# georghess/neurad-studio

Measured on NVIDIA H100. Metric: rays/sec (camera+lidar), higher is better.
Workload: dtype f32

## Files before the change

### neurad-studio_b200/csrc/b200nerf.cu

```cuda
#include <cuda_runtime.h>

#include <cstdio>
#include <cstring>
#include <new>
#include <string>
#include <vector>

#include "../../include/b200nerf.h"
#include "nff_device.h"
#include "nff_lane.h"
#include "rgb_decoder.cuh"
#include "modules.cuh"

using namespace nff;

static thread_local std::string g_err;
static int fail(int code, const std::string& msg) {
  g_err = msg;
  return code;
}
#define CUDA_TRY(expr)                                                                                   \
  do {                                                                                                   \
    cudaError_t e_ = (expr);                                                                             \
    if (e_ != cudaSuccess)                                                                               \
// ... 108 lines not shown
  mlp.stage = reinterpret_cast<float*>(smem_tc + kTcBytes) + group * kTcStageFloats;
  mlp.bar_id = 1 + group;
  const int64_t stride = (int64_t)gridDim.x * WARPS;
  for (int64_t base = (int64_t)blockIdx.x * WARPS; base < P.n_rays; base += stride) {
    const int64_t ray = base + warp;
    const bool active = ray < P.n_rays;
    render_ray(P, *ws, mlp, active ? ray : P.n_rays - 1, active);
  }
}



__device__ __forceinline__ int64_t lane_units(const RenderParams& P) {
  const int W = P.rays.image_width;
  if (W <= 0) return (P.n_rays + kLaneThreads - 1) / kLaneThreads;
  constexpr int kTileH = kLaneThreads / 32;
  const int64_t H = (P.n_rays + W - 1) / W;
  return (int64_t)((W + 31) / 32) * ((H + kTileH - 1) / kTileH);
}
__device__ __forceinline__ bool lane_unit_ray(const RenderParams& P, int64_t unit, int tid, int64_t* ray_out) {
  const int W = P.rays.image_width;
  int64_t ray, fallback;
  bool active;
  if (W > 0) {
    constexpr int kTileH = kLaneThreads / 32;
    const int64_t H = (P.n_rays + W - 1) / W, tiles_x = (W + 31) / 32;
    const int warp = tid >> 5, lane_ = tid & 31;
    const int64_t px = (unit % tiles_x) * 32 + (warp & 3) * 8 + (lane_ & 7);
    const int64_t py = (unit / tiles_x) * kTileH + (warp >> 2) * 4 + (lane_ >> 3);
    ray = py * W + px;
    active = px < W && ray < P.n_rays;
    fallback = (py < H ? py : H - 1) * W + (px < W ? px : W - 1);
  } else {
    ray = unit * kLaneThreads + tid;
    active = ray < P.n_rays;
    fallback = P.n_rays - 1;
  }
  if (fallback >= P.n_rays) fallback = P.n_rays - 1;
  *ray_out = active ? ray : fallback;
  return active;
}

__device__ __forceinline__ int64_t lane_patches(const RenderParams& P) {
  return P.rays.image_width > 0 ? lane_units(P) * (kLaneThreads / 32) : (P.n_rays + 31) / 32;
}
__device__ __forceinline__ bool lane_patch_ray(const RenderParams& P, int64_t patch, int lane_, int64_t* ray_out) {
  constexpr int kPatchesPerUnit = kLaneThreads / 32;
  return lane_unit_ray(P, patch / kPatchesPerUnit, (int)(patch % kPatchesPerUnit) * 32 + lane_, ray_out);
}

#ifndef NFF_SAMPLE_CTAS
#define NFF_SAMPLE_CTAS 2
#endif
template <int LAYOUT>
__global__ void __launch_bounds__(kLaneThreads, NFF_SAMPLE_CTAS) nff_sample_lane_kernel(const __grid_constant__ RenderParams P,
                                                                                        float* __restrict__ scratch,
                                                                                        float* __restrict__ handoff) {
  const int tid = threadIdx.x, warp = __shfl_sync(0xffffffffu, (int)(threadIdx.x >> 5), 0), lane_ = tid & 31;
  const LaneScratch sc = lane_scratch_of(scratch, blockIdx.x);
  constexpr int kPPU = kLaneThreads / 32;
  const int64_t n_patches = lane_patches(P);
  const int64_t full_rounds = n_patches / kPPU / gridDim.x;
  const int64_t r0 = full_rounds * gridDim.x * kPPU, rest = n_patches - r0;
  const int64_t p0 = r0 + rest * blockIdx.x / gridDim.x, p1 = r0 + rest * (blockIdx.x + 1) / gridDim.x;
  for (int64_t it = 0;; ++it) {
    int64_t patch;
    if (it < full_rounds) {
      patch = (it * gridDim.x + blockIdx.x) * kPPU + warp;
    } else {
      patch = p0 + warp + (it - full_rounds) * kPPU;
      if (patch >= p1) break;
    }
    int64_t ray;
    const bool active = lane_patch_ray(P, patch, lane_, &ray);
    const LaneRay R = lane_ray_setup(P, sc, tid, ray);
    float* col = active ? handoff + ray : sc.bins2 + tid;
    sample_ray_lane<LAYOUT>(P, sc, R, tid, ray, active, col, active ? P.n_rays : (int64_t)kLaneThreads);
  }
}

template <int LAYOUT>
__global__ void __launch_bounds__(kLaneThreads, kLaneCtasPerSm) nff_shade_lane_kernel(const __grid_constant__ RenderParams P,
                                                                                      float* __restrict__ scratch,
                                                                                      const float* __restrict__ handoff) {
  extern __shared__ __align__(128) unsigned char smem_shade[];
  TcShared* tcs = reinterpret_cast<TcShared*>(smem_shade);
  const int tid = threadIdx.x, warp = __shfl_sync(0xffffffffu, (int)(threadIdx.x >> 5), 0), group = warp >> 2;
  tc_stage_weights(*tcs, P.main_mlp_nn, tid, kLaneThreads, true);
  tc::fence_async_smem();
  __syncthreads();
  MlpLaneTc mlp;
  mlp.t = tcs;
  mlp.panel_ = reinterpret_cast<float*>(smem_shade + kTcBytes);
  mlp.bar_id = 1 + group;
  const LaneScratch sc = lane_scratch_of(scratch, blockIdx.x);
  mlp.sh_tcnn = LAYOUT;
  constexpr int kPPU = kLaneThreads / 32;
  const int64_t n_patches = lane_patches(P);
  const int64_t full_rounds = n_patches / kPPU / gridDim.x;
  const int64_t r0 = full_rounds * gridDim.x * kPPU;
  const int64_t rest_groups = (n_patches - r0 + 3) / 4;
  const int64_t g0 = rest_groups * blockIdx.x / gridDim.x, g1 = rest_groups * (blockIdx.x + 1) / gridDim.x;
  for (int64_t it = 0;; ++it) {
    int64_t patch;
    if (it < full_rounds) {
      patch = (it * gridDim.x + blockIdx.x) * kPPU + warp;
    } else {
      const int64_t gu = g0 + group + (it - full_rounds) * (kLaneThreads / 128);
      if (gu >= g1) break;
      patch = r0 + gu * 4 + (warp & 3);
    }
    int64_t ray;
    const bool active = lane_patch_ray(P, patch, tid & 31, &ray);
    const LaneRay R = lane_ray_setup(P, sc, tid, ray);
    shade_ray_lane<MlpLaneTc, LAYOUT>(P, sc, R, mlp, tid, ray, active, handoff + ray, P.n_rays);
  }
}

__global__ void __launch_bounds__(kLaneThreads, kLaneCtasPerSm) nff_render_lane_kernel(const __grid_constant__ RenderParams P,
                                                                          float* __restrict__ scratch) {
  extern __shared__ __align__(128) unsigned char smem_lane[];
  TcShared* tcs = reinterpret_cast<TcShared*>(smem_lane);
  const int tid = threadIdx.x, warp = __shfl_sync(0xffffffffu, (int)(threadIdx.x >> 5), 0), group = warp >> 2;
  tc_stage_weights(*tcs, P.main_mlp_nn, tid, kLaneThreads, true);
  tc::fence_async_smem();
  __syncthreads();
  MlpLaneTc mlp;
  mlp.t = tcs;
  mlp.panel_ = reinterpret_cast<float*>(smem_lane + kTcBytes);
  mlp.bar_id = 1 + group;
  const LaneScratch sc = lane_scratch_of(scratch, blockIdx.x);
// ... 634 lines not shown
static void offset_rays(RenderParams& Q, int64_t start, int fdim) {
  if (start == 0) return;
  adv(Q.rays.origins, 3 * start); adv(Q.rays.directions, 3 * start); adv(Q.rays.pixel_area, start);
  adv(Q.rays.times, start); adv(Q.rays.nears, start); adv(Q.rays.fars, start);
  adv(Q.rays.sensor_idx, start); adv(Q.rays.is_lidar, start);
  adv(Q.out.features, (int64_t)fdim * start); adv(Q.out.depth, start); adv(Q.out.accumulation, start);
  adv(Q.out.prop_depth_0, start); adv(Q.out.prop_depth_1, start);
  b200nerf_trace& t = Q.trace;
  adv(t.prop_weights_0, kS0 * start); adv(t.prop_weights_1, kS1 * start);
  adv(t.bins_s_1, (kS1 + 1) * start); adv(t.bins_e_1, (kS1 + 1) * start);
  adv(t.bins_s_2, (kS2 + 1) * start); adv(t.bins_e_2, (kS2 + 1) * start);
  adv(t.inds_1, (kS1 + 1) * start); adv(t.inds_2, (kS2 + 1) * start);
  adv(t.sdf, kS2 * start); adv(t.alpha, kS2 * start); adv(t.field_feature, (int64_t)kS2 * kNff * start);
  adv(t.weights, kS2 * start);
  adv(t.actor_id_0, kS0 * start); adv(t.actor_id_1, kS1 * start); adv(t.actor_id_main, kS2 * start);
  Q.peers.row_offset += start;
}


extern "C" {

const char* b200nerf_last_error(void) { return g_err.c_str(); }
int b200nerf_version(void) { return B200NERF_VERSION; }

int b200nerf_create(int device_ordinal, b200nerf_ctx** out) {
  REQUIRE(out != nullptr, "out is NULL");
  int n = 0;
  CUDA_TRY(cudaGetDeviceCount(&n));
  REQUIRE(device_ordinal >= 0 && device_ordinal < n, "device ordinal out of range");
  DeviceGuard g(device_ordinal);
  cudaDeviceProp prop;
  CUDA_TRY(cudaGetDeviceProperties(&prop, device_ordinal));
  if (prop.major != 9 || prop.minor != 0)
    return fail(B200NERF_ERR_UNSUPPORTED, "libb200nerf is built for sm_90a only (found sm_" +
                                              std::to_string(prop.major) + std::to_string(prop.minor) + ")");
  b200nerf_ctx* c = new (std::nothrow) b200nerf_ctx();
  REQUIRE(c != nullptr, "out of host memory");
  c->device = device_ordinal;
  c->sm_count = prop.multiProcessorCount;
  CUDA_TRY(cudaFuncSetAttribute(nff_render_kernel<kRenderWarps>, cudaFuncAttributeMaxDynamicSharedMemorySize,
                                (int)((kMainMlpFloats * 4 + 15) / 16 * 16 + kRenderWarps * sizeof(WarpShared))));
  CUDA_TRY(cudaFuncSetAttribute(nff_render_tc_kernel<kRenderWarps>, cudaFuncAttributeMaxDynamicSharedMemorySize,
                                (int)(tc_smem_bytes(kRenderWarps * 32) + kRenderWarps * sizeof(WarpSharedTc))));
  CUDA_TRY(cudaMalloc((void**)&c->d_status, sizeof(int)));
  CUDA_TRY(cudaMemset(c->d_status, 0, sizeof(int)));
  CUDA_TRY(cudaFuncSetAttribute(nff_render_lane_kernel, cudaFuncAttributeMaxDynamicSharedMemorySize,
                                (int)lane_tc_smem_bytes()));
  c->lane_ctas = c->sm_count * (kLaneCtasPerSm > NFF_SAMPLE_CTAS ? kLaneCtasPerSm : NFF_SAMPLE_CTAS);
  CUDA_TRY(cudaMalloc((void**)&c->d_lane_scratch, sizeof(float) * lane_scratch_floats_per_cta() * c->lane_ctas));
  CUDA_TRY(cudaFuncSetAttribute(nff_shade_lane_kernel<0>, cudaFuncAttributeMaxDynamicSharedMemorySize,
                                (int)lane_tc_smem_bytes()));
  CUDA_TRY(cudaFuncSetAttribute(nff_shade_lane_kernel<1>, cudaFuncAttributeMaxDynamicSharedMemorySize,
                                (int)lane_tc_smem_bytes()));
  CUDA_TRY(cudaFuncSetAttribute(nff_sample_lane_kernel<0>, cudaFuncAttributePreferredSharedMemoryCarveout, 0));
  CUDA_TRY(cudaFuncSetAttribute(nff_sample_lane_kernel<1>, cudaFuncAttributePreferredSharedMemoryCarveout, 0));
  CUDA_TRY(cudaMalloc((void**)&c->d_minmax, 2 * sizeof(unsigned)));
  c->handoff_rays = (int64_t)1 << 21;
  CUDA_TRY(cudaMalloc((void**)&c->d_handoff, sizeof(float) * (kS2 + 1) * c->handoff_rays));
  CUDA_TRY(cudaMalloc((void**)&c->d_grad_actor_ptrs, sizeof(float*) * kModMaxActors));
  *out = c;
  return 0;
}

int b200nerf_destroy(b200nerf_ctx* c) {
  if (!c) return 0;
  DeviceGuard g(c->device);
  for (int i = 0; i < 3; ++i) {
    cudaFree((void*)c->d_actor_tables[i]);
    cudaFree(c->d_decoder[i]);
  }
  cudaFree(c->d_main_mlp);
  cudaFree(c->d_main_mlp_nn);
  cudaFree(c->d_lane_scratch);
  cudaFree(c->d_grad_actor_ptrs);
  cudaFree(c->d_handoff);
  cudaFree(c->d_minmax);
  cudaFree(c->d_lidar_mlp);
  cudaFree(c->d_act_times);
  cudaFree(c->d_act_kf);
  cudaFree(c->d_act_bounds);
  cudaFree(c->d_act_radii);
  cudaFree(c->d_act_present);
  cudaFree(c->d_u1);
  cudaFree(c->d_u2);
  cudaFree(c->d_status);
  for (int i = 0; i < 8; ++i) {
    cudaFree(c->d_dec_wimg[i]);
    cudaFree(c->d_dec_wf32[i]);
  }
  cudaFree(c->d_dec_bias);
  cudaFree(c->d_dec_small);
  delete c;
  return 0;
}

int b200nerf_set_field_grids(b200nerf_ctx* c, int field, const b200nerf_grid_desc* sd, const float* stable,
                             const b200nerf_grid_desc* ad, const float* const* atabs_host, int n_actors,
                             float static_scale, float actor_scale) {
  REQUIRE(c, "ctx is NULL");
  REQUIRE(field >= 0 && field < 3, "field selector out of range");
  REQUIRE(stable != nullptr, "static table is NULL");
  DeviceGuard g(c->device);
  FieldGrids fg{};
  if (int e = make_grid(sd, stable, &fg.stat)) return e;
  const int wantL = field == B200NERF_FIELD_MAIN ? 8 : 6, wantF = field == B200NERF_FIELD_MAIN ? 4 : 1;
  if (fg.stat.L != wantL || fg.stat.F != wantF)
    return fail(B200NERF_ERR_UNSUPPORTED,
                "fused kernel is specialised for NeuRAD's grid shapes (main: 8 levels x 4 features, proposal: 6 x 1)");
// ... 234 lines not shown
    int f = c->samp.field_of_round[i];
    if (!c->have_field[f] || !c->fields[f].decoder)
      return fail(B200NERF_ERR_STATE, "proposal field used by a sampling round has no grids / decoder set");
    if (c->actors.n_actors > 0 && !c->fields[f].actor_tables && !c->fields[f].act.table)
      return fail(B200NERF_ERR_STATE, "actors are set but a proposal field has no actor grids");
  }
  if (c->actors.n_actors > 0 && !c->fields[0].actor_tables && !c->fields[0].act.table)
    return fail(B200NERF_ERR_STATE, "actors are set but the main field has no actor grids");
  if (n_rays == 0) return 0;
  REQUIRE(rays->origins && rays->directions && rays->pixel_area && rays->times, "NULL ray tensor");
  REQUIRE(out->features && out->depth && out->accumulation && out->prop_depth_0 && out->prop_depth_1, "NULL output tensor");
  if ((out->intensity || out->ray_drop_logit) && !c->have_lidar)
    return fail(B200NERF_ERR_STATE, "intensity requested but set_lidar_decoder was not called");
  DeviceGuard g(c->device);
  RenderParams P{};
  for (int i = 0; i < 3; ++i) P.fields[i] = c->fields[i];
  P.main_mlp = c->d_main_mlp;
  P.main_mlp_nn = c->d_main_mlp_nn;
  P.status = c->d_status;
  P.lidar_mlp = c->d_lidar_mlp;
  P.beta = c->beta;
  P.nff_dim = kNff;
  P.actors = c->actors;
  P.samp = c->samp;
  P.app = c->app;
  P.rays = *rays;
  P.out = *out;
  if (trace) P.trace = *trace;
  P.peers = c->peers;
  if (c->peers.n_peers > 0 && c->mlp_mode < 2)
    return fail(B200NERF_ERR_UNSUPPORTED, "peer outputs are implemented by the ray-per-lane kernels (modes 2, 3) only");
  if (c->peers.n_peers > 0 && ((kNff + c->app.dim) & 3) != 0)
    return fail(B200NERF_ERR_UNSUPPORTED, "peer outputs need a feature width that is a multiple of 4");
  P.n_rays = n_rays;
  P.layout = c->layout;
  if (c->layout == 1) {
    if (c->mlp_mode != 3)
      return fail(B200NERF_ERR_UNSUPPORTED, "the tiny-cuda-nn layout is implemented by the two-stage renderer (mode 3) only");
    for (int i = 0; i < 2; ++i)
      if (c->field_layout[c->samp.field_of_round[i]] != 1)
        return fail(B200NERF_ERR_STATE, "main field has the tiny-cuda-nn layout but a proposal field used for sampling does not");
  } else {
    for (int i = 0; i < 2; ++i)
      if (c->field_layout[c->samp.field_of_round[i]] != 0)
        return fail(B200NERF_ERR_STATE, "a proposal field has the tiny-cuda-nn layout but the main field does not");
  }
  constexpr int WARPS = kRenderWarps;
  int64_t blocks_needed = (n_rays + WARPS - 1) / WARPS;
  int64_t max_blocks = (int64_t)c->sm_count * (16 / WARPS);
  int blocks = (int)(blocks_needed < max_blocks ? blocks_needed : max_blocks);
  cudaStream_t st = (cudaStream_t)stream;
  if (c->mlp_mode == 3) {
    const size_t smem = lane_tc_smem_bytes();
    int64_t slice = c->handoff_rays;
    if (rays->image_width > 0) {
      const int64_t band = (int64_t)rays->image_width * (kLaneThreads / 32);
      REQUIRE(band <= slice, "image_width too large for the two-stage renderer");
      slice = slice / band * band;
    }
    const int fdim = kNff + c->app.dim;
    for (int64_t start = 0; start < n_rays; start += slice) {
      const int64_t cnt = n_rays - start < slice ? n_rays - start : slice;
      RenderParams Q = P;
      Q.n_rays = cnt;
      offset_rays(Q, start, fdim);
      int64_t need = (cnt + kLaneThreads - 1) / kLaneThreads;
      if (rays->image_width > 0) {
        const int64_t W = rays->image_width, H = (cnt + W - 1) / W;
        need = ((W + 31) / 32) * ((H + kLaneThreads / 32 - 1) / (kLaneThreads / 32));
      }
      const int64_t max_a = (int64_t)c->sm_count * NFF_SAMPLE_CTAS, max_b = (int64_t)c->sm_count * kLaneCtasPerSm;
      const int64_t patches = rays->image_width > 0 ? need * (kLaneThreads / 32) : (cnt + 31) / 32, groups = (patches + 3) / 4;
      const int64_t grid_a = patches < max_a ? patches : max_a, grid_b = groups < max_b ? groups : max_b;
      if (c->layout == 1) {
        nff_sample_lane_kernel<1><<<(int)grid_a, kLaneThreads, 0, st>>>(Q, c->d_lane_scratch, c->d_handoff);
        nff_shade_lane_kernel<1><<<(int)grid_b, kLaneThreads, smem, st>>>(Q, c->d_lane_scratch, c->d_handoff);
      } else {
        nff_sample_lane_kernel<0><<<(int)grid_a, kLaneThreads, 0, st>>>(Q, c->d_lane_scratch, c->d_handoff);
        nff_shade_lane_kernel<0><<<(int)grid_b, kLaneThreads, smem, st>>>(Q, c->d_lane_scratch, c->d_handoff);
      }
    }
  } else if (c->mlp_mode == 2) {
    const size_t smem = lane_tc_smem_bytes();
    int64_t need = (n_rays + kLaneThreads - 1) / kLaneThreads;
    if (rays->image_width > 0) {
      const int64_t W = rays->image_width, H = (n_rays + W - 1) / W;
      need = ((W + 31) / 32) * ((H + kLaneThreads / 32 - 1) / (kLaneThreads / 32));
    }
    int lane_blocks = (int)(need < c->lane_ctas ? need : c->lane_ctas);
    nff_render_lane_kernel<<<lane_blocks, kLaneThreads, smem, st>>>(P, c->d_lane_scratch);
  } else if (c->mlp_mode == 1) {
    const size_t smem = tc_smem_bytes(WARPS * 32) + WARPS * sizeof(WarpSharedTc);
    nff_render_tc_kernel<WARPS><<<blocks, WARPS * 32, smem, st>>>(P);
  } else {
    const size_t smem = (kMainMlpFloats * 4 + 15) / 16 * 16 + WARPS * sizeof(WarpShared);
    nff_render_kernel<WARPS><<<blocks, WARPS * 32, smem, st>>>(P);
  }
  CUDA_TRY(cudaGetLastError());
  if (out->intensity || out->ray_drop_logit) {
    int fdim = kNff + c->app.dim;
    lidar_decode_kernel<<<(unsigned)((n_rays + 127) / 128), 128, 0, st>>>(c->d_lidar_mlp, out->features, fdim, n_rays,
                                                                          out->intensity, out->ray_drop_logit);
    CUDA_TRY(cudaGetLastError());
  }
  return 0;
}


static int mlp_fwd_impl(b200nerf_ctx* c, const float* x, int64_t n_rows, int in_dim, int n_layers,
                        const float* const* weights_host, const float* const* biases_host, const int* out_dims_host,
                        float* y, float* const* hidden_pre_host, void* stream, const float* relu_mask = nullptr);
int b200nerf_mlp_fwd(b200nerf_ctx* c, const float* x, int64_t n_rows, int in_dim, int n_layers,
                     const float* const* weights_host, const float* const* biases_host, const int* out_dims_host,
                     float* y, void* stream) {
  return mlp_fwd_impl(c, x, n_rows, in_dim, n_layers, weights_host, biases_host, out_dims_host, y, nullptr, stream);
}
int b200nerf_mlp_fwd_train(b200nerf_ctx* c, const float* x, int64_t n_rows, int in_dim, int n_layers,
                           const float* const* weights_host, const float* const* biases_host, const int* out_dims_host,
                           float* y, float* const* hidden_pre_host, void* stream) {
  return mlp_fwd_impl(c, x, n_rows, in_dim, n_layers, weights_host, biases_host, out_dims_host, y, hidden_pre_host, stream);
}
int b200nerf_mlp_dgrad(b200nerf_ctx* c, const float* dy, int64_t n_rows, int dy_dim, const float* weight_t, int dx_dim,
                       const float* relu_z, float* dx, void* stream) {
  const float* w[1] = {weight_t};
  const int od[1] = {dx_dim};
  return mlp_fwd_impl(c, dy, n_rows, dy_dim, 1, w, nullptr, od, dx, nullptr, stream, relu_z);
}
static int mlp_fwd_impl(b200nerf_ctx* c, const float* x, int64_t n_rows, int in_dim, int n_layers,
                        const float* const* weights_host, const float* const* biases_host, const int* out_dims_host,
                        float* y, float* const* hidden_pre_host, void* stream, const float* relu_mask) {
  REQUIRE(c && weights_host && out_dims_host, "NULL argument");
// ... 876 lines not shown
```

### neurad-studio_b200/csrc/nff_device.h

```cpp
#pragma once
#include "nff_params.h"
#include "simt.h"

#ifndef NFF_G_PROP
#define NFF_G_PROP 1
#endif
#ifndef NFF_G_ACT
#define NFF_G_ACT 2
#endif
#ifndef NFF_ILP
#define NFF_ILP 2
#endif
#ifndef NFF_F4_UNROLL
#define NFF_F4_UNROLL 2
#endif
#ifndef NFF_FAST_RCP
#define NFF_FAST_RCP 1
#endif
#ifndef NFF_PARITY_STD
#define NFF_PARITY_STD 0
#endif
#ifndef NFF_PARITY_LERP
#define NFF_PARITY_LERP 0
#endif
#define NFF_STR2(x) #x
#define NFF_STR(x) NFF_STR2(x)

namespace nff {
using namespace simt;
constexpr int kF4Unroll = NFF_F4_UNROLL;

NFF_D float nan_to_num(float v) {
  if (v != v) return 0.0f;
  if (v > 3.4028234663852886e38f) return 3.4028234663852886e38f;
  if (v < -3.4028234663852886e38f) return -3.4028234663852886e38f;
  return v;
}
NFF_D float warp_sum(float v) {
#pragma unroll
  for (int m = 16; m >= 1; m >>= 1) v += shfl_xor(v, m);
  return v;
}
NFF_D float warp_scan_add(float v) {
#pragma unroll
  for (int d = 1; d < 32; d <<= 1) {
    float n = shfl_up(v, d);
    if (lane() >= d) v += n;
  }
  return v;
}
NFF_D float warp_scan_mul(float v) {
#pragma unroll
  for (int d = 1; d < 32; d <<= 1) {
    float n = shfl_up(v, d);
    if (lane() >= d) v *= n;
  }
  return v;
}

NFF_D float pow_lam(float t, float e) { return e == -1.0f ? frcp(t) : powf(t, e); }
NFF_D float spacing_fn(float x, const Sampling& s) {
  float t = fadd(fdiv(fmul(x, s.scaling), s.lam_1), 1.0f);
  return fmul(s.ratio, fsub(pow_lam(t, s.lam), 1.0f));
}
NFF_D float spacing_fn_inv(float y, const Sampling& s) {
  float t = fadd(fdiv(fmul(y, s.lam), s.lam_1), 1.0f);
  t = fmaxf(t, 1e-10f);
  float r = fmul(fsub(pow_lam(t, s.lam == -1.0f ? -1.0f : 1.0f / s.lam), 1.0f), s.lam_1);
  return fdiv(r, s.scaling);
}
NFF_D float to_euclid(float u, float s_near, float s_far, const Sampling& s) {
  return spacing_fn_inv(fadd(fmul(u, s_far), fmul(fsub(1.0f, u), s_near)), s);
}
NFF_D float linspace01(int i, int n) {
  float step = fdiv(1.0f, (float)n);
  return i < (n + 1) / 2 ? fmul(step, (float)i) : fsub(1.0f, fmul(step, (float)(n - i)));
}

struct Gauss {
  float x, y, z, std;
};
NFF_D Gauss sample_gaussian(const float o[3], const float d[3], float area, float start, float end) {
  float md = fdiv(fsub(end, start), 2.0f);
  float t = fadd(start, md);
  Gauss g;
  g.x = fadd(o[0], fmul(d[0], t));
  g.y = fadd(o[1], fmul(d[1], t));
  g.z = fadd(o[2], fmul(d[2], t));
  float cs = fmul(area, fmul(t, t));
#if NFF_PARITY_STD
  g.std = powf(fmul(cs, md), 0.33333334f);
#else
  g.std = cbrtf(fmul(cs, md));
#endif
  return g;
}
NFF_D Gauss contract(Gauss g, float scale) {
  float x = fdiv(g.x, scale), y = fdiv(g.y, scale), z = fdiv(g.z, scale);
#if NFF_PARITY_STD
  float sd = fdiv(g.std, scale);
#else
  float sd = fmul(g.std, frcp(scale));
#endif
  float mag = fmaxf(fmaxf(fabsf(x), fabsf(y)), fabsf(z));
  if (!(mag < 1.0f)) {
    const float a = fsub(2.0f, frcp(mag));
    x = fmul(a, fdiv(x, mag));
    y = fmul(a, fdiv(y, mag));
    z = fmul(a, fdiv(z, mag));
#if NFF_PARITY_STD
    float q = fdiv(powf(fsub(fmul(2.0f, mag), 1.0f), 0.33333334f), mag);
#else
    float q = fmul(cbrtf(fsub(fmul(2.0f, mag), 1.0f)), frcp(mag));
#endif
    sd = fmul(sd, fmul(q, q));
  }
  Gauss r;
  r.x = fmul(fadd(x, 2.0f), 0.25f);
// ... 853 lines not shown
```

### neurad-studio_b200/csrc/nff_lane.h

```cpp
#pragma once
#include "nff_device.h"

namespace nff {

#ifndef NFF_LANE_THREADS
#define NFF_LANE_THREADS 512
#endif
#ifndef NFF_F4_WEIGHTS
#define NFF_F4_WEIGHTS 0
#endif
constexpr int kLaneThreads = NFF_LANE_THREADS;
constexpr int kLaneCtasPerSm = 512 / kLaneThreads;
constexpr int kCandFloats = 16;
constexpr int kLaneMaxCand = 32;

struct LaneScratch {
  float* w;
  float* bins1;
  float* bins2;
  float* cand;
};
NFF_HD size_t lane_scratch_floats_per_cta() {
  return (size_t)kLaneThreads * (kS0 + (kS1 + 1) + (kS2 + 1) + kLaneMaxCand * kCandFloats);
}
// ... 35 lines not shown
    float v[3] = {fsub(p[6], o[0]), fsub(p[7], o[1]), fsub(p[8], o[2])};
    float cx = fsub(fmul(v[1], d[2]), fmul(v[2], d[1]));
    float cy = fsub(fmul(v[2], d[0]), fmul(v[0], d[2]));
    float cz = fsub(fmul(v[0], d[1]), fmul(v[1], d[0]));
    float dist = fsqrt(fadd(fadd(fmul(cx, cx), fmul(cy, cy)), fmul(cz, cz)));
    if (!(valid && dist < ldg(A.radii + a) * 1.001f)) continue;
    if (n >= kLaneMaxCand) {
      *overflow = 1;
      continue;
    }
    float b1[3] = {p[0], p[1], p[2]};
    normalize3(b1);
    float dt = fadd(fadd(fmul(b1[0], p[3]), fmul(b1[1], p[4])), fmul(b1[2], p[5]));
    float b2[3] = {fsub(p[3], fmul(dt, b1[0])), fsub(p[4], fmul(dt, b1[1])), fsub(p[5], fmul(dt, b1[2]))};
    normalize3(b2);
    float b3[3] = {fsub(fmul(b1[1], b2[2]), fmul(b1[2], b2[1])), fsub(fmul(b1[2], b2[0]), fmul(b1[0], b2[2])),
                   fsub(fmul(b1[0], b2[1]), fmul(b1[1], b2[0]))};
    float R[9] = {b1[0], b2[0], b3[0], b1[1], b2[1], b3[1], b1[2], b2[2], b3[2]};
    float* c = sc.cand + (size_t)n * kCandFloats * kLaneThreads + tid;
#pragma unroll
    for (int i = 0; i < 3; ++i) {
      c[(4 * i + 0) * kLaneThreads] = R[3 * i + 0];
      c[(4 * i + 1) * kLaneThreads] = R[3 * i + 1];
      c[(4 * i + 2) * kLaneThreads] = R[3 * i + 2];
      c[(4 * i + 3) * kLaneThreads] = -fadd(fadd(fmul(R[3 * i], p[6]), fmul(R[3 * i + 1], p[7])), fmul(R[3 * i + 2], p[8]));
      c[(12 + i) * kLaneThreads] = ldg(A.bounds + 3 * a + i);
    }
    c[15 * kLaneThreads] = (float)a;
    ++n;
  }
  return n;
}

NFF_D int lane_actor_of_sample(const LaneScratch& sc, int tid, int n_cand, const Gauss& g, float pb[3], float M_out[12]) {
  int hit = -1;
  for (int c = 0; c < n_cand; ++c) {
    const float* p = sc.cand + (size_t)c * kCandFloats * kLaneThreads + tid;
    float M[12];
#pragma unroll
    for (int i = 0; i < 12; ++i) M[i] = p[i * kLaneThreads];
    float q0 = fadd(fadd(fadd(fmul(M[0], g.x), fmul(M[1], g.y)), fmul(M[2], g.z)), M[3]);
    float q1 = fadd(fadd(fadd(fmul(M[4], g.x), fmul(M[5], g.y)), fmul(M[6], g.z)), M[7]);
    float q2 = fadd(fadd(fadd(fmul(M[8], g.x), fmul(M[9], g.y)), fmul(M[10], g.z)), M[11]);
    if (fabsf(q0) < p[12 * kLaneThreads] && fabsf(q1) < p[13 * kLaneThreads] && fabsf(q2) < p[14 * kLaneThreads]) {
      hit = (int)p[15 * kLaneThreads];
      pb[0] = q0; pb[1] = q1; pb[2] = q2;
#pragma unroll
      for (int i = 0; i < 12; ++i) M_out[i] = M[i];
    }
  }
  return hit;
}

template <int LAYOUT = 0>
NFF_D float lane_proposal_density(const FieldGrids& fg, const LaneScratch& sc, int tid, int n_cand, const Gauss& g,
                                  int* actor_id) {
  float pb[3], M[12];
  int a = n_cand > 0 ? lane_actor_of_sample(sc, tid, n_cand, g, pb, M) : -1;
  float acc;
  if (a >= 0) {
    Gauss ga = {pb[0], pb[1], pb[2], g.std};
    ga = contract(ga, fg.actor_scale);
    if (LAYOUT == 1) {
      const float x4[4] = {ga.x, ga.y, ga.z, fdiv((float)a, fg.n_actors_f)};
      acc = tcnn_encode_f1_dot<4>(fg.act, 4, x4, ga.std, fg.decoder);
    } else {
      acc = encode_f1_dot<4, NFF_G_ACT>(fg.actor_tables[a], fg.act, ga, fg.decoder);
    }
  } else {
    Gauss gs = contract(g, fg.static_scale);
    if (LAYOUT == 1) {
      const float x3[3] = {gs.x, gs.y, gs.z};
      acc = tcnn_encode_f1_dot<3>(fg.stat, 6, x3, gs.std, fg.decoder);
    } else {
      acc = encode_f1_dot<6, NFF_G_PROP>(fg.stat.table, fg.stat, gs, fg.decoder);
    }
  }
  *actor_id = a;
  return expf(acc);
}

NFF_D void encode_f4_col(const float* NFF_RESTRICT table, const Grid& gr, int L, Gauss g, float* x , int pitch) {
  const uint32_t maskb = gr.mask << 4;
#pragma unroll 2
  for (int l = 0; l < L; ++l) {
    const float res = gr.res[l];
    const CellB<4> c = grid_cell_b<4>(g.x, g.y, g.z, res);
    uint32_t r[8];
    cell_offsets_b<4>(c, maskb, r);
    const char* base = level_base(table, l, gr.T, 16);
    float4 v[8];
#pragma unroll
    for (int k = 0; k < 8; ++k) v[k] = ldg_at<float4>(base, r[k]);
    float w = level_weight(res, g.std);
    const float ix = 1.0f - c.ox, iy = 1.0f - c.oy, iz = 1.0f - c.oz;
#if NFF_F4_WEIGHTS
    const float z1 = c.oz * w, z0 = iz * w;
    const float y1z1 = c.oy * z1, y0z1 = iy * z1, y1z0 = c.oy * z0, y0z0 = iy * z0;
    const float wk[8] = {c.ox * y1z1, c.ox * y0z1, ix * y0z1, ix * y1z1, c.ox * y1z0, c.ox * y0z0, ix * y0z0, ix * y1z0};
    float a0 = wk[0] * v[0].x, a1 = wk[0] * v[0].y, a2 = wk[0] * v[0].z, a3 = wk[0] * v[0].w;
#pragma unroll
    for (int k = 1; k < 8; ++k) {
      a0 = fmaf(wk[k], v[k].x, a0);
      a1 = fmaf(wk[k], v[k].y, a1);
      a2 = fmaf(wk[k], v[k].z, a2);
      a3 = fmaf(wk[k], v[k].w, a3);
    }
    x[(4 * l + 0) * pitch] = a0;
    x[(4 * l + 1) * pitch] = a1;
    x[(4 * l + 2) * pitch] = a2;
    x[(4 * l + 3) * pitch] = a3;
#else
    float f[8];
#pragma unroll
    for (int k = 0; k < 8; ++k) f[k] = v[k].x;
    x[(4 * l + 0) * pitch] = fmul(trilerp_b<4>(f, c, ix, iy, iz), w);
#pragma unroll
    for (int k = 0; k < 8; ++k) f[k] = v[k].y;
    x[(4 * l + 1) * pitch] = fmul(trilerp_b<4>(f, c, ix, iy, iz), w);
#pragma unroll
    for (int k = 0; k < 8; ++k) f[k] = v[k].z;
    x[(4 * l + 2) * pitch] = fmul(trilerp_b<4>(f, c, ix, iy, iz), w);
#pragma unroll
    for (int k = 0; k < 8; ++k) f[k] = v[k].w;
    x[(4 * l + 3) * pitch] = fmul(trilerp_b<4>(f, c, ix, iy, iz), w);
#endif
  }
}

struct LaneRoundIO {
  int S, S_new;
  const float* u_tab;
  float* bins_out;
  int64_t bins_stride;
  float* tr_w;
  int32_t* tr_aid;
  float* tr_bins_s;
  float* tr_bins_e;
  int32_t* tr_inds;
};
template <int LAYOUT = 0>
NFF_D float lane_proposal_round(const RenderParams& P, const FieldGrids& fg, const LaneScratch& sc, int tid, int n_cand,
                                const LaneRoundIO& io, const float* bins_in, const float o[3], const float d[3], float area,
                                float s_near, float s_far, int64_t ray) {
  const Sampling& sp = P.samp;
  const int S = io.S, S_new = io.S_new;
  auto edge = [bins_in, S](int i) { return bins_in ? bins_in[(size_t)i * kLaneThreads] : linspace01(i, S); };
  double excl = 0.0, tot_d = 0.0;
  float depth_acc = 0.0f;
  float e_prev = to_euclid(edge(0), s_near, s_far, sp);
#pragma unroll 1
  for (int s = 0; s < S; ++s) {
    const float T = expf(-(float)excl);
    float w = 0.0f;
    if (!(vote_all_converged(T == 0.0f) && io.tr_aid == nullptr)) {
      const float e0 = e_prev;
      const float e1 = to_euclid(edge(s + 1), s_near, s_far, sp);
      e_prev = e1;
      Gauss g = sample_gaussian(o, d, area, e0, e1);
      int aid;
      float dens = lane_proposal_density<LAYOUT>(fg, sc, tid, n_cand, g, &aid);
      float dd = fmul(fsub(e1, e0), dens);
      float alpha = fsub(1.0f, expf(-dd));
      excl += (double)dd;
      w = nan_to_num(fmul(alpha, T));
      depth_acc = fadd(depth_acc, fmul(w, fmul(fadd(e0, e1), 0.5f)));
      if (io.tr_aid) io.tr_aid[ray * S + s] = aid;
    }
    if (io.tr_w) io.tr_w[ray * S + s] = w;
    w = fadd(w, sp.hist_pad);
    sc.w[(size_t)s * kLaneThreads + tid] = w;
    tot_d += (double)w;
  }
  float tot = (float)tot_d;
  const float padding = fmaxf(fsub(1e-5f, tot), 0.0f);
  const float pad_each = fdiv(padding, (float)S);
  tot = fadd(tot, padding);
  int k = 1;
  double run = (double)fdiv(fadd(sc.w[tid], pad_each), tot);
  float c_km1 = 0.0f, c_k = fminf(1.0f, (float)run);
  float w_next = sc.w[(size_t)kLaneThreads + tid];
#pragma unroll 1
  for (int i = 0; i <= S_new; ++i) {
    const float u = ldg(io.u_tab + i);
    while (k <= S && c_k <= u) {
      ++k;
      c_km1 = c_k;
      if (k <= S) {
        const float wk = w_next;
        w_next = sc.w[(size_t)(k < S ? k : S - 1) * kLaneThreads + tid];
        run += (double)fdiv(fadd(wk, pad_each), tot);
        c_k = fminf(1.0f, (float)run);
      }
    }
    const int above = k > S ? S : k;
    const float b0 = edge(k - 1), b1 = edge(above);
    float t = nan_to_num(fdiv(fsub(u, c_km1), fsub(k > S ? c_km1 : c_k, c_km1)));
    t = fminf(fmaxf(t, 0.0f), 1.0f);
    const float nb = fadd(b0, fmul(t, fsub(b1, b0)));
    io.bins_out[(size_t)i * io.bins_stride] = nb;
    if (io.tr_inds) io.tr_inds[ray * (S_new + 1) + i] = k;
    if (io.tr_bins_s) io.tr_bins_s[ray * (S_new + 1) + i] = nb;
    if (io.tr_bins_e) io.tr_bins_e[ray * (S_new + 1) + i] = to_euclid(nb, s_near, s_far, sp);
  }
  return depth_acc;
}

struct MlpLaneFfma {
  static constexpr int kPitch = kLaneThreads;
  const float* w;
  float* panel_;
  int sh_tcnn = 0;
  NFF_D float* panel() const { return panel_; }
  NFF_D void run(const float* x, const float dir[3], float& sdf, float* feat, int ) const {
    float h[kHidden], go[kNff + 1], in2[kNff + kSh], h2[kHidden];
    dense<kGeoIn, kHidden, kHidden, true>(w + kOffGeoW0, w + kOffGeoB0, x, h);
    dense<kHidden, kNff + 1, kGeoOutP, false>(w + kOffGeoW1, w + kOffGeoB1, h, go);
    sdf = go[0];
#pragma unroll
    for (int i = 0; i < kNff; ++i) in2[i] = go[i + 1];
    if (sh_tcnn) sh4_tcnn(dir[0], dir[1], dir[2], in2 + kNff); else sh4(dir[0], dir[1], dir[2], in2 + kNff);
    dense<kNff + kSh, kHidden, kHidden, true>(w + kOffFeatW0, w + kOffFeatB0, in2, h);
    dense<kHidden, kHidden, kHidden, true>(w + kOffFeatW1, w + kOffFeatB1, h, h2);
    dense<kHidden, kNff, kNff, false>(w + kOffFeatW2, w + kOffFeatB2, h2, h);
#pragma unroll
    for (int i = 0; i < kNff; ++i) feat[i] = in2[i] + h[i];
  }
};

#if defined(__CUDACC__)
constexpr int kLanePanelPitch = kLaneThreads + 8;
constexpr int kLanePanelRows = kGeoIn + kSh + 1;
constexpr size_t lane_tc_smem_bytes() { return (size_t)kTcBytes + sizeof(float) * kLanePanelRows * kLanePanelPitch; }
struct MlpLaneTc {
  static constexpr int kPitch = kLanePanelPitch;
  const TcShared* t;
  float* panel_;
  int bar_id;
  int sh_tcnn = 0;
  NFF_D float* panel() const { return panel_; }
  NFF_D void group_sync() const { asm volatile("bar.sync %0, 128;" ::"r"(bar_id) : "memory"); }

  template <int KS, int K>
  NFF_D static void half_mma(float* acc, const float* a, const float* b_hi) {
    uint32_t ah[4 * KS], al[4 * KS];
#pragma unroll
    for (int i = 0; i < 4 * KS; ++i) {
      const float h = tc::tf32_hi(a[i]);
      ah[i] = __float_as_uint(h);
      al[i] = __float_as_uint(a[i] - h);
    }
    const uint32_t sbo = (uint32_t)(K / 4) * 128u;
    const uint64_t dh = tc::smem_desc(tc::smem_u32(b_hi), 128u, sbo), dl = tc::smem_desc(tc::smem_u32(b_hi + 32 * K), 128u, sbo);
    tc::wg_fence();
#pragma unroll
    for (int ks = 0; ks < KS; ++ks) {
// ... 70 lines not shown
      s1 += __shfl_xor_sync(0xffffffffu, s1, 1);
      s0 += __shfl_xor_sync(0xffffffffu, s0, 2);
      s1 += __shfl_xor_sync(0xffffffffu, s1, 2);
      if (q == 0) {
        p[(kGeoIn + kSh) * kPitch] = s0 + t->b_sdf;
        p[(kGeoIn + kSh) * kPitch + 8] = s1 + t->b_sdf;
      }
      chain(a, acc);
      bias_init(acc, t->bias[1], q);
      half_mma<4, 32>(acc, a, t->b + tc_layer_off(1));
      __syncwarp();
#pragma unroll
      for (int j = 0; j < 4; ++j) {
        float* r = p + (8 * j + 2 * q) * kPitch;
        r[0] = acc[4 * j + 0], r[kPitch] = acc[4 * j + 1], r[8] = acc[4 * j + 2], r[kPitch + 8] = acc[4 * j + 3];
      }
      chain(a, acc);
      bias_init(acc, t->bias[2], q);
      half_mma<4, 48>(acc, a, t->b + tc_layer_off(2));
      load_a(a, p, q, 4, 2);
      half_mma<2, 48>(acc, a, t->b + tc_layer_off(2) + 4 * 64);
      relu(acc);
      chain(a, acc);
      bias_init(acc, t->bias[3], q);
      half_mma<4, 32>(acc, a, t->b + tc_layer_off(3));
      relu(acc);
      chain(a, acc);
      bias_init(acc, t->bias[4], q);
#pragma unroll
      for (int j = 0; j < 4; ++j) {
        const float* r = p + (8 * j + 2 * q) * kPitch;
        acc[4 * j + 0] += r[0], acc[4 * j + 1] += r[kPitch], acc[4 * j + 2] += r[8], acc[4 * j + 3] += r[kPitch + 8];
      }
      half_mma<4, 32>(acc, a, t->b + tc_layer_off(4));
#pragma unroll
      for (int j = 0; j < 4; ++j) {
        float* r = p + (8 * j + 2 * q) * kPitch;
        r[0] = acc[4 * j + 0], r[kPitch] = acc[4 * j + 1], r[8] = acc[4 * j + 2], r[kPitch + 8] = acc[4 * j + 3];
      }
    }
    group_sync();
#pragma unroll
    for (int i = 0; i < kNff; ++i) feat[i] = col[i * kPitch];
    sdf = col[(kGeoIn + kSh) * kPitch];
  }
};
#endif

struct LaneRay {
  float o[3], d[3];
  float area, time, s_near, s_far;
  int n_cand;
};
NFF_D LaneRay lane_ray_setup(const RenderParams& P, const LaneScratch& sc, int tid, int64_t ray) {
  const Sampling& sp = P.samp;
  LaneRay R;
#pragma unroll
  for (int i = 0; i < 3; ++i) {
    R.o[i] = ldg(P.rays.origins + 3 * ray + i);
    R.d[i] = ldg(P.rays.directions + 3 * ray + i);
  }
  const bool lidar = P.rays.is_lidar ? P.rays.is_lidar[ray] != 0 : false;
  R.area = fmul(ldg(P.rays.pixel_area + ray), lidar ? 1.0f : sp.cam_area_scale);
  R.time = ldg(P.rays.times + ray);
  float far_ = P.rays.fars ? ldg(P.rays.fars + ray) : 1.0e6f;
  far_ = fminf(far_, sp.sky_distance);
  const float near_ = P.rays.nears ? ldg(P.rays.nears + ray) : 0.0f;
  R.s_near = spacing_fn(near_, sp);
  R.s_far = spacing_fn(far_, sp);
  int overflow = 0;
  R.n_cand = lane_actor_candidates(P.actors, R.time, R.o, R.d, sc, tid, &overflow);
#if defined(__CUDACC__)
  if (overflow && P.status) atomicExch(P.status, 3);
#endif
  return R;
}

template <int LAYOUT = 0>
NFF_D void sample_ray_lane(const RenderParams& P, const LaneScratch& sc, const LaneRay& R, int tid, int64_t ray, bool active,
                           float* bins2, int64_t bins2_stride) {
  const Sampling& sp = P.samp;
  float prop_depth[2];
#pragma unroll 1
  for (int rd = 0; rd < 2; ++rd) {
    LaneRoundIO io;
    io.S = rd == 0 ? kS0 : kS1;
    io.S_new = rd == 0 ? kS1 : kS2;
    io.u_tab = rd == 0 ? sp.u1 : sp.u2;
    io.bins_out = rd == 0 ? sc.bins1 + tid : bins2;
    io.bins_stride = rd == 0 ? (int64_t)kLaneThreads : bins2_stride;
    io.tr_w = !active ? nullptr : rd == 0 ? P.trace.prop_weights_0 : P.trace.prop_weights_1;
    io.tr_aid = !active ? nullptr : rd == 0 ? P.trace.actor_id_0 : P.trace.actor_id_1;
    io.tr_bins_s = !active ? nullptr : rd == 0 ? P.trace.bins_s_1 : P.trace.bins_s_2;
    io.tr_bins_e = !active ? nullptr : rd == 0 ? P.trace.bins_e_1 : P.trace.bins_e_2;
    io.tr_inds = !active ? nullptr : rd == 0 ? P.trace.inds_1 : P.trace.inds_2;
    prop_depth[rd] = lane_proposal_round<LAYOUT>(P, P.fields[sp.field_of_round[rd]], sc, tid, R.n_cand, io,
                                         rd == 0 ? nullptr : sc.bins1 + tid, R.o, R.d, R.area, R.s_near, R.s_far, ray);
  }
  if (active) {
    P.out.prop_depth_0[ray] = prop_depth[0];
    P.out.prop_depth_1[ray] = prop_depth[1];
  }
}

template <class Mlp, int LAYOUT = 0>
NFF_D void shade_ray_lane(const RenderParams& P, const LaneScratch& sc, const LaneRay& R, Mlp& mlp, int tid, int64_t ray,
                          bool active, const float* bins2, int64_t bins2_stride) {
  const Sampling& sp = P.samp;
  const float* o = R.o;
  const float* d = R.d;
  const float area = R.area, time = R.time, s_near = R.s_near, s_far = R.s_far;
  const int n_cand = R.n_cand;

  const FieldGrids& fm = P.fields[B200NERF_FIELD_MAIN];
  float fsum[kNff];
#pragma unroll
  for (int i = 0; i < kNff; ++i) fsum[i] = 0.0f;
  double T_d = 1.0;
  float acc = 0.0f, depth = 0.0f;
  float e_prev = to_euclid(bins2[0], s_near, s_far, sp);
#pragma unroll 1
  for (int s = 0; s < kS2; ++s) {
    const float e0 = e_prev;
    float e1 = to_euclid(bins2[(size_t)(s + 1) * bins2_stride], s_near, s_far, sp);
    e_prev = e1;
    if (s == kS2 - 1) e1 = fadd(e1, fsub(sp.sky_distance, e1));
    Gauss g = sample_gaussian(o, d, area, e0, e1);
    float* col = mlp.panel() + tid;
    float dir[3] = {d[0], d[1], d[2]};
    int aid = -1;
    {
      float pb[3], M[12];
      aid = n_cand > 0 ? lane_actor_of_sample(sc, tid, n_cand, g, pb, M) : -1;
      if (aid >= 0) {
        Gauss ga = {pb[0], pb[1], pb[2], g.std};
        ga = contract(ga, fm.actor_scale);
#pragma unroll
        for (int i = 16; i < 32; ++i) col[i * Mlp::kPitch] = 0.0f;
        if (LAYOUT == 1) {
          const float x4[4] = {ga.x, ga.y, ga.z, fdiv((float)aid, fm.n_actors_f)};
          tcnn_encode_f4<4>(fm.act, 4, x4, ga.std, col, Mlp::kPitch);
        } else {
          encode_f4_col(fm.actor_tables[aid], fm.act, 4, ga, col, Mlp::kPitch);
        }
        float q0 = fadd(fadd(fmul(M[0], d[0]), fmul(M[1], d[1])), fmul(M[2], d[2]));
        float q1 = fadd(fadd(fmul(M[4], d[0]), fmul(M[5], d[1])), fmul(M[6], d[2]));
        float q2 = fadd(fadd(fmul(M[8], d[0]), fmul(M[9], d[1])), fmul(M[10], d[2]));
        float n = fadd(fsqrt(fadd(fadd(fmul(q0, q0), fmul(q1, q1)), fmul(q2, q2))), 1.0e-7f);
        dir[0] = fdiv(q0, n); dir[1] = fdiv(q1, n); dir[2] = fdiv(q2, n);
      } else {
        Gauss gs = contract(g, fm.static_scale);
        if (LAYOUT == 1) {
          const float x3[3] = {gs.x, gs.y, gs.z};
          tcnn_encode_f4<3>(fm.stat, 8, x3, gs.std, col, Mlp::kPitch);
// ... 117 lines not shown
```

Before: 79.02 million.

## Specialize sample kernel on actors/tracing and precompute shared round-0 edges

Templates the sampling kernel on whether actors exist and whether trace outputs are requested, and picks the instantiation on the host, so the no-actor, no-trace path drops candidate tests and trace-store branches. When rays have no per-ray near/far, the round-0 Euclidean bin edges are the same for every ray, so they are computed once per block into shared memory instead of per ray per sample. It also adds a fast path in the inverse spacing function for lam == -1 that uses a reciprocal instead of a pow. The cost is more kernel instantiations (more compile time and code size) and a per-block shared table plus barrier.

```diff
diff --git a/neurad-studio_b200/csrc/b200nerf.cu b/neurad-studio_b200/csrc/b200nerf.cu
--- a/neurad-studio_b200/csrc/b200nerf.cu
+++ b/neurad-studio_b200/csrc/b200nerf.cu
@@ -184,12 +184,18 @@
 #ifndef NFF_SAMPLE_CTAS
 #define NFF_SAMPLE_CTAS 2
 #endif
-template <int LAYOUT>
+template <int LAYOUT, bool ACTORS, bool TRACED>
 __global__ void __launch_bounds__(kLaneThreads, NFF_SAMPLE_CTAS) nff_sample_lane_kernel(const __grid_constant__ RenderParams P,
                                                                                         float* __restrict__ scratch,
                                                                                         float* __restrict__ handoff) {
   const int tid = threadIdx.x, warp = __shfl_sync(0xffffffffu, (int)(threadIdx.x >> 5), 0), lane_ = tid & 31;
   const LaneScratch sc = lane_scratch_of(scratch, blockIdx.x);
+  __shared__ float e0_tab[kS0 + 1];
+  const bool shared_edges = !P.rays.nears && !P.rays.fars;
+  if (shared_edges) {
+    if (tid <= kS0) e0_tab[tid] = lane_round0_edge(P.samp, tid);
+    __syncthreads();
+  }
   constexpr int kPPU = kLaneThreads / 32;
   const int64_t n_patches = lane_patches(P);
   const int64_t full_rounds = n_patches / kPPU / gridDim.x;
@@ -205,10 +211,17 @@
     }
     int64_t ray;
     const bool active = lane_patch_ray(P, patch, lane_, &ray);
-    const LaneRay R = lane_ray_setup(P, sc, tid, ray);
+    const LaneRay R = lane_ray_setup<ACTORS>(P, sc, tid, ray);
     float* col = active ? handoff + ray : sc.bins2 + tid;
-    sample_ray_lane<LAYOUT>(P, sc, R, tid, ray, active, col, active ? P.n_rays : (int64_t)kLaneThreads);
-  }
+    sample_ray_lane<LAYOUT, ACTORS, TRACED>(P, sc, R, tid, ray, active, col, active ? P.n_rays : (int64_t)kLaneThreads,
+                                            shared_edges ? e0_tab : nullptr);
+  }
+}
+template <int LAYOUT>
+static auto sample_lane_kernel(bool actors, bool traced) {
+  return traced ? nff_sample_lane_kernel<LAYOUT, true, true>
+         : actors ? nff_sample_lane_kernel<LAYOUT, true, false>
+                  : nff_sample_lane_kernel<LAYOUT, false, false>;
 }
 
 template <int LAYOUT>
@@ -949,8 +962,10 @@
                                 (int)lane_tc_smem_bytes()));
   CUDA_TRY(cudaFuncSetAttribute(nff_shade_lane_kernel<1>, cudaFuncAttributeMaxDynamicSharedMemorySize,
                                 (int)lane_tc_smem_bytes()));
-  CUDA_TRY(cudaFuncSetAttribute(nff_sample_lane_kernel<0>, cudaFuncAttributePreferredSharedMemoryCarveout, 0));
-  CUDA_TRY(cudaFuncSetAttribute(nff_sample_lane_kernel<1>, cudaFuncAttributePreferredSharedMemoryCarveout, 0));
+  for (int i = 0; i < 4; ++i) {
+    CUDA_TRY(cudaFuncSetAttribute(sample_lane_kernel<0>(i & 1, i & 2), cudaFuncAttributePreferredSharedMemoryCarveout, 0));
+    CUDA_TRY(cudaFuncSetAttribute(sample_lane_kernel<1>(i & 1, i & 2), cudaFuncAttributePreferredSharedMemoryCarveout, 0));
+  }
   CUDA_TRY(cudaMalloc((void**)&c->d_minmax, 2 * sizeof(unsigned)));
   c->handoff_rays = (int64_t)1 << 21;
   CUDA_TRY(cudaMalloc((void**)&c->d_handoff, sizeof(float) * (kS2 + 1) * c->handoff_rays));
@@ -1291,6 +1306,9 @@
   cudaStream_t st = (cudaStream_t)stream;
   if (c->mlp_mode == 3) {
     const size_t smem = lane_tc_smem_bytes();
+    const b200nerf_trace& tr = P.trace;
+    const bool traced = tr.prop_weights_0 || tr.prop_weights_1 || tr.actor_id_0 || tr.actor_id_1 || tr.bins_s_1 ||
+                        tr.bins_s_2 || tr.bins_e_1 || tr.bins_e_2 || tr.inds_1 || tr.inds_2;
     int64_t slice = c->handoff_rays;
     if (rays->image_width > 0) {
       const int64_t band = (int64_t)rays->image_width * (kLaneThreads / 32);
@@ -1311,11 +1329,12 @@
       const int64_t max_a = (int64_t)c->sm_count * NFF_SAMPLE_CTAS, max_b = (int64_t)c->sm_count * kLaneCtasPerSm;
       const int64_t patches = rays->image_width > 0 ? need * (kLaneThreads / 32) : (cnt + 31) / 32, groups = (patches + 3) / 4;
       const int64_t grid_a = patches < max_a ? patches : max_a, grid_b = groups < max_b ? groups : max_b;
+      const bool actors = c->actors.n_actors > 0;
       if (c->layout == 1) {
-        nff_sample_lane_kernel<1><<<(int)grid_a, kLaneThreads, 0, st>>>(Q, c->d_lane_scratch, c->d_handoff);
+        sample_lane_kernel<1>(actors, traced)<<<(int)grid_a, kLaneThreads, 0, st>>>(Q, c->d_lane_scratch, c->d_handoff);
         nff_shade_lane_kernel<1><<<(int)grid_b, kLaneThreads, smem, st>>>(Q, c->d_lane_scratch, c->d_handoff);
       } else {
-        nff_sample_lane_kernel<0><<<(int)grid_a, kLaneThreads, 0, st>>>(Q, c->d_lane_scratch, c->d_handoff);
+        sample_lane_kernel<0>(actors, traced)<<<(int)grid_a, kLaneThreads, 0, st>>>(Q, c->d_lane_scratch, c->d_handoff);
         nff_shade_lane_kernel<0><<<(int)grid_b, kLaneThreads, smem, st>>>(Q, c->d_lane_scratch, c->d_handoff);
       }
     }
diff --git a/neurad-studio_b200/csrc/nff_device.h b/neurad-studio_b200/csrc/nff_device.h
--- a/neurad-studio_b200/csrc/nff_device.h
+++ b/neurad-studio_b200/csrc/nff_device.h
@@ -64,6 +64,10 @@
   return fmul(s.ratio, fsub(pow_lam(t, s.lam), 1.0f));
 }
 NFF_D float spacing_fn_inv(float y, const Sampling& s) {
+  if (s.lam == -1.0f) {
+    const float t = fmaxf(fadd(fmul(y, -0.5f), 1.0f), 1e-10f);
+    return fdiv(fmul(fsub(frcp(t), 1.0f), s.lam_1), s.scaling);
+  }
   float t = fadd(fdiv(fmul(y, s.lam), s.lam_1), 1.0f);
   t = fmaxf(t, 1e-10f);
   float r = fmul(fsub(pow_lam(t, s.lam == -1.0f ? -1.0f : 1.0f / s.lam), 1.0f), s.lam_1);
diff --git a/neurad-studio_b200/csrc/nff_lane.h b/neurad-studio_b200/csrc/nff_lane.h
--- a/neurad-studio_b200/csrc/nff_lane.h
+++ b/neurad-studio_b200/csrc/nff_lane.h
@@ -111,11 +111,11 @@
   return hit;
 }
 
-template <int LAYOUT = 0>
+template <int LAYOUT = 0, bool ACTORS = true>
 NFF_D float lane_proposal_density(const FieldGrids& fg, const LaneScratch& sc, int tid, int n_cand, const Gauss& g,
                                   int* actor_id) {
   float pb[3], M[12];
-  int a = n_cand > 0 ? lane_actor_of_sample(sc, tid, n_cand, g, pb, M) : -1;
+  int a = ACTORS && n_cand > 0 ? lane_actor_of_sample(sc, tid, n_cand, g, pb, M) : -1;
   float acc;
   if (a >= 0) {
     Gauss ga = {pb[0], pb[1], pb[2], g.std};
@@ -198,35 +198,36 @@
   float* tr_bins_e;
   int32_t* tr_inds;
 };
-template <int LAYOUT = 0>
+template <int LAYOUT = 0, bool ACTORS = true, bool TRACED = true>
 NFF_D float lane_proposal_round(const RenderParams& P, const FieldGrids& fg, const LaneScratch& sc, int tid, int n_cand,
-                                const LaneRoundIO& io, const float* bins_in, const float o[3], const float d[3], float area,
-                                float s_near, float s_far, int64_t ray) {
+                                const LaneRoundIO& io, const float* bins_in, const float* e_tab, const float o[3],
+                                const float d[3], float area, float s_near, float s_far, int64_t ray) {
   const Sampling& sp = P.samp;
   const int S = io.S, S_new = io.S_new;
   auto edge = [bins_in, S](int i) { return bins_in ? bins_in[(size_t)i * kLaneThreads] : linspace01(i, S); };
+  auto euclid = [&](int i) { return e_tab ? e_tab[i] : to_euclid(edge(i), s_near, s_far, sp); };
   double excl = 0.0, tot_d = 0.0;
   float depth_acc = 0.0f;
-  float e_prev = to_euclid(edge(0), s_near, s_far, sp);
+  float e_prev = euclid(0);
 #pragma unroll 1
   for (int s = 0; s < S; ++s) {
     const float T = expf(-(float)excl);
     float w = 0.0f;
-    if (!(vote_all_converged(T == 0.0f) && io.tr_aid == nullptr)) {
+    if (!(vote_all_converged(T == 0.0f) && (!TRACED || io.tr_aid == nullptr))) {
       const float e0 = e_prev;
-      const float e1 = to_euclid(edge(s + 1), s_near, s_far, sp);
+      const float e1 = euclid(s + 1);
       e_prev = e1;
       Gauss g = sample_gaussian(o, d, area, e0, e1);
       int aid;
-      float dens = lane_proposal_density<LAYOUT>(fg, sc, tid, n_cand, g, &aid);
+      float dens = lane_proposal_density<LAYOUT, ACTORS>(fg, sc, tid, n_cand, g, &aid);
       float dd = fmul(fsub(e1, e0), dens);
       float alpha = fsub(1.0f, expf(-dd));
       excl += (double)dd;
       w = nan_to_num(fmul(alpha, T));
       depth_acc = fadd(depth_acc, fmul(w, fmul(fadd(e0, e1), 0.5f)));
-      if (io.tr_aid) io.tr_aid[ray * S + s] = aid;
-    }
-    if (io.tr_w) io.tr_w[ray * S + s] = w;
+      if (TRACED && io.tr_aid) io.tr_aid[ray * S + s] = aid;
+    }
+    if (TRACED && io.tr_w) io.tr_w[ray * S + s] = w;
     w = fadd(w, sp.hist_pad);
     sc.w[(size_t)s * kLaneThreads + tid] = w;
     tot_d += (double)w;
@@ -258,9 +259,9 @@
     t = fminf(fmaxf(t, 0.0f), 1.0f);
     const float nb = fadd(b0, fmul(t, fsub(b1, b0)));
     io.bins_out[(size_t)i * io.bins_stride] = nb;
-    if (io.tr_inds) io.tr_inds[ray * (S_new + 1) + i] = k;
-    if (io.tr_bins_s) io.tr_bins_s[ray * (S_new + 1) + i] = nb;
-    if (io.tr_bins_e) io.tr_bins_e[ray * (S_new + 1) + i] = to_euclid(nb, s_near, s_far, sp);
+    if (TRACED && io.tr_inds) io.tr_inds[ray * (S_new + 1) + i] = k;
+    if (TRACED && io.tr_bins_s) io.tr_bins_s[ray * (S_new + 1) + i] = nb;
+    if (TRACED && io.tr_bins_e) io.tr_bins_e[ray * (S_new + 1) + i] = to_euclid(nb, s_near, s_far, sp);
   }
   return depth_acc;
 }
@@ -437,6 +438,17 @@
   float area, time, s_near, s_far;
   int n_cand;
 };
+constexpr float kDefaultNear = 0.0f, kDefaultFar = 1.0e6f;
+NFF_D void lane_spacing_bounds(const Sampling& sp, float near_, float far_, float* s_near, float* s_far) {
+  *s_near = spacing_fn(near_, sp);
+  *s_far = spacing_fn(fminf(far_, sp.sky_distance), sp);
+}
+NFF_D float lane_round0_edge(const Sampling& sp, int i) {
+  float s_near, s_far;
+  lane_spacing_bounds(sp, kDefaultNear, kDefaultFar, &s_near, &s_far);
+  return to_euclid(linspace01(i, kS0), s_near, s_far, sp);
+}
+template <bool ACTORS = true>
 NFF_D LaneRay lane_ray_setup(const RenderParams& P, const LaneScratch& sc, int tid, int64_t ray) {
   const Sampling& sp = P.samp;
   LaneRay R;
@@ -448,43 +460,40 @@
   const bool lidar = P.rays.is_lidar ? P.rays.is_lidar[ray] != 0 : false;
   R.area = fmul(ldg(P.rays.pixel_area + ray), lidar ? 1.0f : sp.cam_area_scale);
   R.time = ldg(P.rays.times + ray);
-  float far_ = P.rays.fars ? ldg(P.rays.fars + ray) : 1.0e6f;
-  far_ = fminf(far_, sp.sky_distance);
-  const float near_ = P.rays.nears ? ldg(P.rays.nears + ray) : 0.0f;
-  R.s_near = spacing_fn(near_, sp);
-  R.s_far = spacing_fn(far_, sp);
+  const float far_ = P.rays.fars ? ldg(P.rays.fars + ray) : kDefaultFar;
+  const float near_ = P.rays.nears ? ldg(P.rays.nears + ray) : kDefaultNear;
+  lane_spacing_bounds(sp, near_, far_, &R.s_near, &R.s_far);
   int overflow = 0;
-  R.n_cand = lane_actor_candidates(P.actors, R.time, R.o, R.d, sc, tid, &overflow);
+  R.n_cand = ACTORS ? lane_actor_candidates(P.actors, R.time, R.o, R.d, sc, tid, &overflow) : 0;
 #if defined(__CUDACC__)
   if (overflow && P.status) atomicExch(P.status, 3);
 #endif
   return R;
 }
 
-template <int LAYOUT = 0>
+template <int LAYOUT = 0, bool ACTORS = true, bool TRACED = true>
 NFF_D void sample_ray_lane(const RenderParams& P, const LaneScratch& sc, const LaneRay& R, int tid, int64_t ray, bool active,
-                           float* bins2, int64_t bins2_stride) {
+                           float* bins2, int64_t bins2_stride, const float* e0_tab = nullptr) {
   const Sampling& sp = P.samp;
-  float prop_depth[2];
 #pragma unroll 1
   for (int rd = 0; rd < 2; ++rd) {
-    LaneRoundIO io;
+    LaneRoundIO io{};
     io.S = rd == 0 ? kS0 : kS1;
     io.S_new = rd == 0 ? kS1 : kS2;
     io.u_tab = rd == 0 ? sp.u1 : sp.u2;
     io.bins_out = rd == 0 ? sc.bins1 + tid : bins2;
     io.bins_stride = rd == 0 ? (int64_t)kLaneThreads : bins2_stride;
-    io.tr_w = !active ? nullptr : rd == 0 ? P.trace.prop_weights_0 : P.trace.prop_weights_1;
-    io.tr_aid = !active ? nullptr : rd == 0 ? P.trace.actor_id_0 : P.trace.actor_id_1;
-    io.tr_bins_s = !active ? nullptr : rd == 0 ? P.trace.bins_s_1 : P.trace.bins_s_2;
-    io.tr_bins_e = !active ? nullptr : rd == 0 ? P.trace.bins_e_1 : P.trace.bins_e_2;
-    io.tr_inds = !active ? nullptr : rd == 0 ? P.trace.inds_1 : P.trace.inds_2;
-    prop_depth[rd] = lane_proposal_round<LAYOUT>(P, P.fields[sp.field_of_round[rd]], sc, tid, R.n_cand, io,
-                                         rd == 0 ? nullptr : sc.bins1 + tid, R.o, R.d, R.area, R.s_near, R.s_far, ray);
-  }
-  if (active) {
-    P.out.prop_depth_0[ray] = prop_depth[0];
-    P.out.prop_depth_1[ray] = prop_depth[1];
+    if (TRACED) {
+      io.tr_w = !active ? nullptr : rd == 0 ? P.trace.prop_weights_0 : P.trace.prop_weights_1;
+      io.tr_aid = !active ? nullptr : rd == 0 ? P.trace.actor_id_0 : P.trace.actor_id_1;
+      io.tr_bins_s = !active ? nullptr : rd == 0 ? P.trace.bins_s_1 : P.trace.bins_s_2;
+      io.tr_bins_e = !active ? nullptr : rd == 0 ? P.trace.bins_e_1 : P.trace.bins_e_2;
+      io.tr_inds = !active ? nullptr : rd == 0 ? P.trace.inds_1 : P.trace.inds_2;
+    }
+    const float prop_depth = lane_proposal_round<LAYOUT, ACTORS, TRACED>(
+        P, P.fields[sp.field_of_round[rd]], sc, tid, R.n_cand, io, rd == 0 ? nullptr : sc.bins1 + tid,
+        rd == 0 ? e0_tab : nullptr, R.o, R.d, R.area, R.s_near, R.s_far, ray);
+    if (active) (rd == 0 ? P.out.prop_depth_0 : P.out.prop_depth_1)[ray] = prop_depth;
   }
 }
 
```

Result: faster. 85.23 million, median of 6 (+7.9%).
